# zhangxinsong-nlp/XFM

Hardware: AMD Instinct MI355X
Metric: image-text pairs/sec fwd+bwd, XFM-base 224px/30tok (higher is better)
Workload: dtype bf16; 1 GPU; Pretrain.py full multimodal step (ITC+ITM+MLM+MIM), XFM-base, synthetic 224px images + 30-token captions, random init; units_per_gpu=64, global_batch=64, dropout=True, ordered_reductions=True, grad_allreduce=False, parallelism=dp1, image_res=224

## Files before the change

xfm_amd/csrc/attention.hip:

```cpp
#include "attention_common.h"
#include "attention_general.hip"
#include "attention_short.hip"
#include "attention_grouped.hip"
#include "attention_vit.hip"
#include "attention_long.hip"
#include "attention_aux.hip"

static int attn_check(const AttnArgs& a, bool bwd) {
  XFM_REQUIRE(a.B > 0 && a.H > 0 && a.Sq > 0 && a.Sk > 0, "attention: empty problem B=%d H=%d Sq=%d Sk=%d", a.B, a.H, a.Sq, a.Sk);
  XFM_REQUIRE(a.q_rs % 8 == 0 && a.k_rs % 8 == 0 && a.v_rs % 8 == 0 && a.o_rs % 4 == 0, "attention: row strides must be multiples of 8");
  XFM_REQUIRE(((uintptr_t)a.q % 16) == 0 && ((uintptr_t)a.k % 16) == 0 && ((uintptr_t)a.v % 16) == 0 && ((uintptr_t)a.o % 8) == 0,
              "attention: q/k/v must be 16-byte aligned");
  XFM_REQUIRE(a.bias == nullptr || (a.bias_ld % 4 == 0 && a.bias_ld >= a.Sk), "attention: bias_ld must be a multiple of 4 and >= Sk");
  XFM_REQUIRE(a.B <= 65535 && a.H <= 65535, "attention: B/H exceed grid limits");
  XFM_REQUIRE(a.stat_ld >= a.Sq && a.stat_ld % 4 == 0 && ((uintptr_t)a.lse % 16) == 0, "attention: stat_ld must be a multiple of 4 and >= Sq, lse 16-byte aligned");
  XFM_REQUIRE(a.bias_t == nullptr || (a.bias != nullptr && a.bias_t_ld % 4 == 0 && a.bias_t_ld >= a.Sq), "attention: bad transposed bias");
  XFM_REQUIRE((a.q_start == nullptr) == (a.q_len == nullptr) && (a.k_start == nullptr) == (a.k_len == nullptr), "attention: packed rows need both start and len");
  XFM_REQUIRE((a.q_start == nullptr && a.k_start == nullptr) || (a.bias == nullptr && a.dbias == nullptr && a.kv_index == nullptr),
              "attention: packed rows take no additive bias and no kv_index");
  if (bwd) {
    XFM_REQUIRE(a.bwd_phase >= 0 && a.bwd_phase <= 2, "attention bwd: bwd_phase must be 0, 1 or 2");
    XFM_REQUIRE(a.dout && a.dq && a.dk && a.dv && a.delta && a.lse, "attention bwd: missing buffers");
    XFM_REQUIRE(a.do_rs % 8 == 0 && a.dq_rs % 4 == 0 && a.dk_rs % 4 == 0 && a.dv_rs % 4 == 0, "attention bwd: bad strides");
  }
  return XFM_OK;
}

static int attn_check_grouped(const AttnArgs& a) {
  XFM_REQUIRE(a.grp_rows != nullptr && a.n_groups > 0 && a.n_groups <= 65535, "grouped attention: grp_rows / n_groups missing");
  XFM_REQUIRE(a.Sq <= 64, "grouped attention needs Sq <= 64 (got %d)", a.Sq);
  XFM_REQUIRE(a.bias == nullptr && a.dbias == nullptr && a.causal == 0 && a.kv_index == nullptr,
              "grouped attention: no bias / causal mask / kv_index (the group index IS the key/value source)");
  XFM_REQUIRE(a.k_start == nullptr && a.k_len == nullptr, "grouped attention: only the query side may be packed (k_start / k_len must be NULL)");
  return XFM_OK;
}

int xfm_attn_fwd_impl(const AttnArgs& a, hipStream_t st) {
  int rc = attn_check(a, false);
  if (rc != XFM_OK) return rc;
  if (a.grp_start != nullptr) {
    rc = attn_check_grouped(a);
    return rc != XFM_OK ? rc : launch_xattn_fwd(a, st);
  }
  if (attn_packable(a)) return launch_xattn_fwd_packed(a, st);
  if (attn_vit_shape(a)) return launch_attn_fwd_vit(a, st);
  return launch_attn_fwd(a, st);
}

__global__ __launch_bounds__(256) void dbias_reduce_kernel(const float* __restrict__ ws, float* __restrict__ dbias, int B, long per_entry) {
  const long e = ((long)blockIdx.x * 256 + threadIdx.x) * 4;
  if (e >= per_entry) return;
  f32x4 acc = *reinterpret_cast<const f32x4*>(dbias + e);
  for (int b = 0; b < B; ++b) acc += *reinterpret_cast<const f32x4*>(ws + (long)b * per_entry + e);
  *reinterpret_cast<f32x4*>(dbias + e) = acc;
}

enum AttnDq { DQ_NONE, DQ_GROUPED, DQ_VIT, DQ_LONG, DQ_SHORT, DQ_SUMS, DQ_GENERAL };
enum AttnDkv { DKV_NONE, DKV_GROUPED, DKV_LONG, DKV_SHORT, DKV_GENERAL };
enum AttnDbias { DB_NONE, DB_ATOMICS, DB_SUMS, DB_ENTRY_WS, DB_SHORT_PLANES, DB_BLOCKS };
struct AttnBwdPlan {
  AttnDq dq;
  AttnDkv dkv;
  AttnDbias dbias;
  int nw, blocks;
  int groups, nb, slices;
  bool pre;
  int planes;
};

static bool xfm_deterministic() { return xfm_env_flag("XFM_DETERMINISTIC", false); }

static AttnBwdPlan attn_bwd_plan(const AttnArgs& a, bool have_ws) {
  AttnBwdPlan p = {};
  const bool run_dq = a.bwd_phase != 2, run_dkv = a.bwd_phase != 1;
  if (a.grp_start != nullptr) {
    if (run_dq) p.dq = DQ_GROUPED;
    if (run_dkv) p.dkv = DKV_GROUPED;
    return p;
  }
  const bool ws_ok = have_ws && a.dbias != nullptr && a.bias_ld % 4 == 0 && a.bias_ld <= (long)cdiv(a.Sk, 64) * 64 && a.q_start == nullptr;
  const int vit_mode = xfm_env_int("XFM_ATTN_VIT_BWD", 0);
  if (attn_vit3_shape(a, vit_mode)) {
    p.dq = DQ_VIT;
    if (a.dbias != nullptr) p.dbias = vit_mode == 4 && attn_dbias_blocks_ok(a) ? DB_BLOCKS : DB_ATOMICS;
  } else if (attn_long_shape(a)) {
    if (run_dq) {
      p.dq = DQ_LONG;
      if (a.dbias != nullptr) p.dbias = DB_BLOCKS;
    }
    if (run_dkv) p.dkv = attn_long_dkv_ok(a) ? DKV_LONG : DKV_GENERAL;
  } else {
    const bool short_ok = attn_short_dq_ok(a);
    attn_geom(a.Sq, p.nw, p.blocks);
    if (run_dq && short_ok) {
      p.dq = DQ_SHORT;
      p.slices = attn_short_dq_slices(a, p.groups, p.nb);
      p.pre = xfm_env_flag("XFM_ATTN_SHORT_PRE", false) && a.o != nullptr && a.o_lo != nullptr;
      if (a.dbias != nullptr) p.dbias = ws_ok && attn_short_planes_ok(a) && p.slices > 1 && xfm_deterministic() ? DB_SHORT_PLANES : DB_ATOMICS;
      if (p.dbias == DB_SHORT_PLANES) p.planes = p.slices;
    } else if (run_dq && a.dbias != nullptr && attn_resident(a.Sk, p.nw) && attn_plain(a)) {
      p.dq = DQ_SUMS;
      p.dbias = DB_SUMS;
      p.nb = attn_dbias_sums_nb(a, p.blocks);
    } else if (run_dq) {
      p.dq = DQ_GENERAL;
      if (a.dbias != nullptr) p.dbias = ws_ok && a.Sk > 64 * ATTN_RES_MAX ? DB_ENTRY_WS : DB_ATOMICS;
      if (p.dbias == DB_ENTRY_WS) p.planes = a.B;
    }
    if (run_dkv) p.dkv = short_ok && a.Sq <= 224 ? DKV_SHORT : DKV_GENERAL;
  }
  if (p.dbias == DB_BLOCKS) {
    p.slices = ws_ok ? attn_dbias_blocks_slices(a) : 1;
    p.planes = p.slices > 1 ? p.slices : 0;
  }
  return p;
}

long xfm_attn_bwd_workspace_impl(const AttnArgs& a) { return (long)attn_bwd_plan(a, true).planes * a.H * a.Sq * a.bias_ld * 4; }

#ifdef XFM_DIAG
static XfmTimeline attn_short_timeline = {nullptr, 0, 0};
static long long* attn_short_stamps(const AttnArgs& a, unsigned workgroups) {
  long long* dbg = a.Sk > 128 && a.Sk <= 224 ? attn_short_timeline.ptr : nullptr;
  if (dbg != nullptr && attn_short_timeline.bytes < (size_t)workgroups * XFM_ATTN_SHORT_STAMP_BYTES) {
    xfm_set_error("attn_bwd_dq_short: timeline buffer of %zu bytes is short of %u workgroups x %d: launched without stamps",
                  attn_short_timeline.bytes, workgroups, XFM_ATTN_SHORT_STAMP_BYTES);
    dbg = nullptr;
  }
  return dbg == nullptr ? dbg : reinterpret_cast<long long*>((uintptr_t)dbg | (uintptr_t)(attn_short_timeline.flags & 15));
}
#endif

int xfm_attn_bwd_impl(const AttnArgs& a_in, hipStream_t st) {
  int rc = attn_check(a_in, true);
  if (rc == XFM_OK && a_in.grp_start != nullptr) rc = attn_check_grouped(a_in);
  if (rc != XFM_OK) return rc;
  const AttnBwdPlan p = attn_bwd_plan(a_in, a_in.dbias_ws != nullptr);
  AttnArgs a = a_in;
  if (p.planes == 0) a.dbias_ws = nullptr;

  switch (p.dq) {
    case DQ_NONE: break;
    case DQ_GROUPED: rc = launch_xattn_dq(a, st); break;
    case DQ_VIT: {
      AttnArgs v = a;
      if (p.dbias == DB_BLOCKS) v.dbias = nullptr;
      rc = launch_attn_bwd_vit3(v, st);
      break;
    }
    case DQ_LONG: rc = launch_attn_bwd_long_dq(a, st); break;
    case DQ_SHORT:
#ifdef XFM_DIAG
      rc = launch_attn_bwd_dq_short(a, p.pre, p.groups, p.nb, p.slices, st, attn_short_stamps(a, (unsigned)(p.groups * a.H * p.slices)));
#else
      rc = launch_attn_bwd_dq_short(a, p.pre, p.groups, p.nb, p.slices, st);
#endif
      break;
    case DQ_SUMS: rc = launch_attn_bwd_dq(a, p.nw, p.blocks, p.nb, st); break;
    case DQ_GENERAL: rc = launch_attn_bwd_dq(a, p.nw, p.blocks, 0, st); break;
  }
  if (rc == XFM_OK && p.dbias == DB_BLOCKS) rc = launch_attn_dbias_blocks(a, p.slices, st);
  if (rc == XFM_OK && p.planes > 0) {
    const long per_entry = (long)a.H * a.Sq * a.bias_ld;
    hipLaunchKernelGGL(dbias_reduce_kernel, dim3(cdiv(per_entry / 4, 256)), dim3(256), 0, st, a.dbias_ws, a.dbias, p.planes, per_entry);
    rc = xfm_check_launch("dbias_reduce");
  }
  if (rc != XFM_OK) return rc;

  switch (p.dkv) {
    case DKV_NONE: break;
    case DKV_GROUPED: rc = launch_xattn_dkv(a, st); break;
    case DKV_LONG: rc = launch_attn_bwd_long_dkv(a, st); break;
    case DKV_SHORT: rc = launch_attn_bwd_dkv_short(a, st); break;
    case DKV_GENERAL: rc = launch_attn_bwd_dkv(a, st); break;
  }
  return rc;
}
```

xfm_amd/csrc/attention_general.hip:

```cpp
template <bool RES, bool PLAIN>
__global__ __launch_bounds__(1024) void attn_fwd_kernel(AttnArgs a) {
  extern __shared__ __attribute__((aligned(16))) char lds[];
  const int tid = threadIdx.x, lane = tid & 63, w = __builtin_amdgcn_readfirstlane(tid >> 6), nthreads = blockDim.x;
  const int lr = lane & 15, lg = lane >> 4;
  const int b = blockIdx.z, h = blockIdx.y;
  long qbase, kbase;
  int sq, sk;
  q_seq(a, b, qbase, sq);
  const int q0 = (blockIdx.x * (nthreads >> 6) + w) * 16;
  const bool wave_active = q0 < sq;
  const int qi = q0 + lr;
  const int qc = qi < sq ? qi : sq - 1;
  const uint32_t dkey = drop_key(a, b, h, qi);
  const bf16* qp = a.q + (qbase + qc) * a.q_rs + h * 64;
  const bf16x8 qf0 = *reinterpret_cast<const bf16x8*>(qp + 8 * lg);
  const bf16x8 qf1 = *reinterpret_cast<const bf16x8*>(qp + 32 + 8 * lg);
  const int kvb = a.kv_index ? a.kv_index[b] : b;
  k_seq(a, kvb, kbase, sk);
  const bf16* kb = a.k + kbase * a.k_rs + h * 64;
  const bf16* vb = a.v + kbase * a.v_rs + h * 64;

  f32x4 oacc[4];
#pragma unroll
  for (int i = 0; i < 4; ++i) oacc[i] = f32x4{0.f, 0.f, 0.f, 0.f};
  float m_run = EXCL_NEG, l_run = 0.f;

  const int nchunks = (sk + 63) / 64;
  constexpr bool resident = RES;
  const int nw = nthreads >> 6;
  if (resident) {
    for (int kc = 0; kc < nchunks; ++kc) stage_slot(lds + kc * ATTN_SLOT, kb, a.k_rs, vb, a.v_rs, kc * 64, sk, w, nw, lane);
    stage_wait();
  } else {
    stage_slot(lds, kb, a.k_rs, vb, a.v_rs, 0, sk, w, nw, lane);
  }
  for (int kc = 0; kc < nchunks; ++kc) {
    if (!resident) {
      stage_wait();
      if (kc + 1 < nchunks) stage_slot(lds + ((kc + 1) & 1) * ATTN_SLOT, kb, a.k_rs, vb, a.v_rs, (kc + 1) * 64, sk, w, nw, lane);
    }
    const char* sK = lds + (resident ? kc : (kc & 1)) * ATTN_SLOT;
    const char* sV = sK + ATTN_TILE;
    if (!wave_active) continue;
    f32x4 st[4], bvs[4];
    int kk[PLAIN ? 1 : 4][4];
    const bool has_mask = !PLAIN && a.key_keep != nullptr;
    const bool causal = !PLAIN && a.causal != 0;
    const bool plain = !has_mask && !causal && kc * 64 + 64 <= sk;
    load_bias(a, h, qc, kc, lg, bvs);
    if constexpr (!PLAIN) {
      if (has_mask) load_keep(a, kvb, kc, lg, kk);
    }
#pragma unroll
    for (int t = 0; t < 4; ++t) {
      st[t] = f32x4{0.f, 0.f, 0.f, 0.f};
      st[t] = __builtin_amdgcn_mfma_f32_16x16x32_bf16(row_frag(sK, t * 16, 0, lr, lg), qf0, st[t], 0, 0, 0);
      st[t] = __builtin_amdgcn_mfma_f32_16x16x32_bf16(row_frag(sK, t * 16, 1, lr, lg), qf1, st[t], 0, 0, 0);
    }
    float mx = EXCL_NEG;
    if (plain) {
#pragma unroll
      for (int t = 0; t < 4; ++t)
#pragma unroll
        for (int r = 0; r < 4; ++r) {
          st[t][r] = fmaf(st[t][r], a.scale, bvs[t][r]);
          mx = fmaxf(mx, st[t][r]);
        }
    } else {
#pragma unroll
      for (int t = 0; t < 4; ++t)
#pragma unroll
        for (int r = 0; r < 4; ++r) {
          st[t][r] = score_masked(a, st[t][r], bvs[t][r], has_mask, has_mask ? kk[PLAIN ? 0 : t][r] : 1, causal, qi, kc * 64 + t * 16 + 4 * lg + r, sk);
          mx = fmaxf(mx, st[t][r]);
        }
    }
    mx = group4_max(mx);
    const float m_new = fmaxf(m_run, mx);
    const float alpha = __expf(m_run - m_new);
    float psum = 0.f;
#pragma unroll
    for (int t = 0; t < 4; ++t)
#pragma unroll
      for (int r = 0; r < 4; ++r) {
        st[t][r] = __expf(st[t][r] - m_new);
        psum += st[t][r];
      }
    if (!PLAIN && a.drop_thresh != 0u) {
#pragma unroll
      for (int t = 0; t < 4; ++t)
#pragma unroll
        for (int r = 0; r < 4; ++r)
          st[t][r] = drop_keep(a, dkey, kc * 64 + t * 16 + 4 * lg + r) ? st[t][r] * a.drop_scale : 0.f;
    }
    psum = group4_sum(psum);
    l_run = l_run * alpha + psum;
    m_run = m_new;
#pragma unroll
    for (int dt = 0; dt < 4; ++dt)
#pragma unroll
      for (int r = 0; r < 4; ++r) oacc[dt][r] *= alpha;
#pragma unroll
    for (int s = 0; s < 2; ++s) {
      const bf16x8 pf = pack_pair(st[2 * s], st[2 * s + 1]);
#pragma unroll
      for (int dt = 0; dt < 4; ++dt)
        oacc[dt] = __builtin_amdgcn_mfma_f32_16x16x32_bf16(tr_frag(sV, 32 * s, 32 * s + 16, dt * 16, lr, lg), pf, oacc[dt], 0, 0, 0);
    }
  }
  if (!wave_active || qi >= sq) return;
  store_out(a, qbase + qi, h, lg, oacc, 1.0f / l_run);
  if (lg == 0) a.lse[((long)b * a.H + h) * a.stat_ld + qi] = m_run + __logf(l_run);
}

template <int NKC, bool RES, bool PLAIN>
__global__ __launch_bounds__(512) void attn_bwd_dq_kernel(AttnArgs a, int nb_per_block) {
  constexpr bool DBIAS = NKC > 0;
  constexpr int NACC = DBIAS ? NKC : 1;
  extern __shared__ __attribute__((aligned(16))) char lds[];
  const int tid = threadIdx.x, lane = tid & 63, w = __builtin_amdgcn_readfirstlane(tid >> 6), nthreads = blockDim.x;
  const int lr = lane & 15, lg = lane >> 4;
  const int h = blockIdx.y;
  const int q0 = (blockIdx.x * (nthreads >> 6) + w) * 16;
  const int qi = q0 + lr;
  constexpr bool resident = RES;

  f32x4 dsacc[NACC][4];
#pragma unroll
  for (int i = 0; i < NACC; ++i)
#pragma unroll
    for (int t = 0; t < 4; ++t) dsacc[i][t] = f32x4{0.f, 0.f, 0.f, 0.f};

  for (int bi = 0; bi < nb_per_block; ++bi) {
    const int b = blockIdx.z * nb_per_block + bi;
    if (b >= a.B) break;
    long qbase, kbase;
    int sq, sk;
    q_seq(a, b, qbase, sq);
    const bool wave_active = q0 < sq;
    const bool qvalid = qi < sq;
    const int qc = qvalid ? qi : sq - 1;
    const uint32_t dkey = drop_key(a, b, h, qi);
    const bf16* qp = a.q + (qbase + qc) * a.q_rs + h * 64;
    const bf16* dop = a.dout + (qbase + qc) * a.do_rs + h * 64;
    const bf16x8 qf0 = *reinterpret_cast<const bf16x8*>(qp + 8 * lg);
    const bf16x8 qf1 = *reinterpret_cast<const bf16x8*>(qp + 32 + 8 * lg);
    const bf16x8 df0 = *reinterpret_cast<const bf16x8*>(dop + 8 * lg);
    const bf16x8 df1 = *reinterpret_cast<const bf16x8*>(dop + 32 + 8 * lg);
    const long stat_idx = ((long)b * a.H + h) * a.stat_ld + qc;
    const float lse = a.lse[stat_idx];
    const int kvb = a.kv_index ? a.kv_index[b] : b;
    k_seq(a, kvb, kbase, sk);
    const int nchunks = (sk + 63) / 64;
    const bf16* kb = a.k + kbase * a.k_rs + h * 64;
    const bf16* vb = a.v + kbase * a.v_rs + h * 64;

    const int nw = nthreads >> 6;
    if (resident) {
      __syncthreads();
      for (int kc = 0; kc < nchunks; ++kc) stage_slot(lds + kc * ATTN_SLOT, kb, a.k_rs, vb, a.v_rs, kc * 64, sk, w, nw, lane);
      stage_wait();
    }
    auto stream_first = [&]() {
      __syncthreads();
      stage_slot(lds, kb, a.k_rs, vb, a.v_rs, 0, sk, w, nw, lane);
    };
    auto stream_next = [&](int kc) {
      stage_wait();
      if (kc + 1 < nchunks) stage_slot(lds + ((kc + 1) & 1) * ATTN_SLOT, kb, a.k_rs, vb, a.v_rs, (kc + 1) * 64, sk, w, nw, lane);
    };
    auto probs = [&](int kc, f32x4 (&st)[4], f32x4 (&dp)[4]) {
      const char* sK = lds + (resident ? kc : (kc & 1)) * ATTN_SLOT;
      const char* sV = sK + ATTN_TILE;
      f32x4 bvs[4];
      int kk[PLAIN ? 1 : 4][4];
      const bool has_mask = !PLAIN && a.key_keep != nullptr;
      const bool causal = !PLAIN && a.causal != 0;
      const bool plain = !has_mask && !causal && kc * 64 + 64 <= sk;
      load_bias(a, h, qc, kc, lg, bvs);
      if constexpr (!PLAIN) {
        if (has_mask) load_keep(a, kvb, kc, lg, kk);
      }
#pragma unroll
      for (int t = 0; t < 4; ++t) {
        st[t] = f32x4{0.f, 0.f, 0.f, 0.f};
        dp[t] = f32x4{0.f, 0.f, 0.f, 0.f};
        st[t] = __builtin_amdgcn_mfma_f32_16x16x32_bf16(row_frag(sK, t * 16, 0, lr, lg), qf0, st[t], 0, 0, 0);
        st[t] = __builtin_amdgcn_mfma_f32_16x16x32_bf16(row_frag(sK, t * 16, 1, lr, lg), qf1, st[t], 0, 0, 0);
        dp[t] = __builtin_amdgcn_mfma_f32_16x16x32_bf16(row_frag(sV, t * 16, 0, lr, lg), df0, dp[t], 0, 0, 0);
        dp[t] = __builtin_amdgcn_mfma_f32_16x16x32_bf16(row_frag(sV, t * 16, 1, lr, lg), df1, dp[t], 0, 0, 0);
      }
      const float lse_q = qvalid ? lse : 3.0e38f;
      if (plain) {
#pragma unroll
        for (int t = 0; t < 4; ++t)
#pragma unroll
          for (int r = 0; r < 4; ++r) st[t][r] = __expf(fmaf(st[t][r], a.scale, bvs[t][r]) - lse_q);
      } else {
#pragma unroll
        for (int t = 0; t < 4; ++t)
#pragma unroll
          for (int r = 0; r < 4; ++r)
            st[t][r] = __expf(score_masked(a, st[t][r], bvs[t][r], has_mask, has_mask ? kk[PLAIN ? 0 : t][r] : 1, causal, qi, kc * 64 + t * 16 + 4 * lg + r, sk) - lse_q);
      }
      if (!PLAIN && a.drop_thresh != 0u) {
#pragma unroll
        for (int t = 0; t < 4; ++t)
#pragma unroll
          for (int r = 0; r < 4; ++r)
            dp[t][r] = drop_keep(a, dkey, kc * 64 + t * 16 + 4 * lg + r) ? dp[t][r] * a.drop_scale : 0.f;
      }
    };

    float delta = 0.f;
    f32x4 st[4], dp[4];
    const bool fast_delta = a.o_lo != nullptr;
    if (fast_delta) {
      delta = delta_from_out(a, qbase + qc, h, lg, df0, df1);
    } else {
      if (!resident) stream_first();
      for (int kc = 0; kc < nchunks; ++kc) {
        if (!resident) stream_next(kc);
        if (wave_active) {
          probs(kc, st, dp);
#pragma unroll
          for (int t = 0; t < 4; ++t)
#pragma unroll
            for (int r = 0; r < 4; ++r) delta += st[t][r] * dp[t][r];
        }
      }
      delta = group4_sum(delta);
    }
    if (wave_active && qvalid && lg == 0) a.delta[stat_idx] = delta;

    f32x4 dqacc[4];
#pragma unroll
    for (int i = 0; i < 4; ++i) dqacc[i] = f32x4{0.f, 0.f, 0.f, 0.f};

    if (!resident && (nchunks > 1 || fast_delta)) stream_first();
    for (int kc = 0; kc < nchunks; ++kc) {
      if (nchunks > 1 || fast_delta) {
        if (!resident) stream_next(kc);
        if (wave_active) probs(kc, st, dp);
      }
      if (!wave_active) continue;
      const char* sK = lds + (resident ? kc : (kc & 1)) * ATTN_SLOT;
      float* wsrow = (!DBIAS && a.dbias != nullptr && a.dbias_ws != nullptr) ? a.dbias_ws + (((long)b * a.H + h) * a.Sq + qi) * a.bias_ld : nullptr;
#pragma unroll
      for (int t = 0; t < 4; ++t) {
        const int kj0 = kc * 64 + t * 16 + 4 * lg;
#pragma unroll
        for (int r = 0; r < 4; ++r) {
          const int kj = kj0 + r;
          const float ds = st[t][r] * (dp[t][r] - delta);
          st[t][r] = ds;
          if (!DBIAS && a.dbias != nullptr && wsrow == nullptr && kj < sk && qvalid) atomicAdd(a.dbias + ((long)h * a.Sq + qi) * a.bias_ld + kj, ds);
        }
        if (!DBIAS && wsrow != nullptr && qvalid) {
          if (kj0 + 4 <= a.bias_ld) *reinterpret_cast<f32x4*>(wsrow + kj0) = st[t];
          else
            for (int r = 0; r < 4; ++r)
              if (kj0 + r < a.bias_ld) wsrow[kj0 + r] = st[t][r];
        }
      }
      if (DBIAS) {
#pragma unroll
        for (int c = 0; c < NACC; ++c)
          if (c == kc) {
#pragma unroll
            for (int t = 0; t < 4; ++t) dsacc[c][t] += st[t];
          }
      }
#pragma unroll
      for (int s2 = 0; s2 < 2; ++s2) {
        const bf16x8 pf = pack_pair(st[2 * s2], st[2 * s2 + 1]);
#pragma unroll
        for (int dt = 0; dt < 4; ++dt)
          dqacc[dt] = __builtin_amdgcn_mfma_f32_16x16x32_bf16(tr_frag(sK, 32 * s2, 32 * s2 + 16, dt * 16, lr, lg), pf, dqacc[dt], 0, 0, 0);
      }
    }
    if (wave_active && qvalid) {
      bf16* dqp = a.dq + (qbase + qi) * a.dq_rs + h * 64;
#pragma unroll
      for (int dt = 0; dt < 4; ++dt) {
        bf16x4 ov;
#pragma unroll
        for (int r = 0; r < 4; ++r) ov[r] = f2bf(dqacc[dt][r] * a.scale);
        *reinterpret_cast<bf16x4*>(dqp + dt * 16 + 4 * lg) = ov;
      }
    }
  }

  if (DBIAS) {
    const bool wave_active = q0 < a.Sq;
    const int nchunks = (a.Sk + 63) / 64;
    float* fl = reinterpret_cast<float*>(lds + w * 4096);
#pragma unroll
    for (int kc = 0; kc < NACC; ++kc) {
      if (kc < nchunks) {
        __syncthreads();
#pragma unroll
        for (int t = 0; t < 4; ++t) *reinterpret_cast<f32x4*>(fl + lr * 64 + t * 16 + 4 * lg) = dsacc[kc][t];
        __syncthreads();
        if (wave_active && a.dbias != nullptr) {
          const int kj = kc * 64 + lane;
          for (int row = 0; row < 16; ++row) {
            const int q = q0 + row;
            if (q < a.Sq && kj < a.Sk) atomicAdd(a.dbias + ((long)h * a.Sq + q) * a.bias_ld + kj, fl[row * 64 + lane]);
          }
        }
      }
    }
  }
}

template <bool RES, bool PLAIN>
__global__ __launch_bounds__(512) void attn_bwd_dkv_kernel(AttnArgs a) {
  extern __shared__ __attribute__((aligned(16))) char lds[];
  const int tid = threadIdx.x, lane = tid & 63, w = __builtin_amdgcn_readfirstlane(tid >> 6), nthreads = blockDim.x;
  const int lr = lane & 15, lg = lane >> 4;
  const int b = blockIdx.z, h = blockIdx.y;
  const int kvb = a.kv_index ? a.kv_index[b] : b;
  long qbase, kbase, kout;
  int sq, sk, sk_unused;
  q_seq(a, b, qbase, sq);
  k_seq(a, kvb, kbase, sk);
  k_seq(a, b, kout, sk_unused);
  const int k0 = (blockIdx.x * (nthreads >> 6) + w) * 16;
  const bool wave_active = k0 < sk;
  const int kj = k0 + lr;
  const bool kvalid = kj < sk;
  const int kcl = kvalid ? kj : sk - 1;
  const bf16* kp = a.k + (kbase + kcl) * a.k_rs + h * 64;
  const bf16* vp = a.v + (kbase + kcl) * a.v_rs + h * 64;
  (void)sk_unused;
  const bf16x8 kf0 = *reinterpret_cast<const bf16x8*>(kp + 8 * lg);
  const bf16x8 kf1 = *reinterpret_cast<const bf16x8*>(kp + 32 + 8 * lg);
  const bf16x8 vf0 = *reinterpret_cast<const bf16x8*>(vp + 8 * lg);
  const bf16x8 vf1 = *reinterpret_cast<const bf16x8*>(vp + 32 + 8 * lg);
  const bf16* qb = a.q + qbase * a.q_rs + h * 64;
  const bf16* db = a.dout + qbase * a.do_rs + h * 64;
  const float* lse_b = a.lse + ((long)b * a.H + h) * a.stat_ld;
  const float* del_b = a.delta + ((long)b * a.H + h) * a.stat_ld;
  bool key_masked = false;
  if (!PLAIN && a.key_keep != nullptr) key_masked = a.key_keep[(long)kvb * a.Sk + kcl] == 0;
  const bool causal = !PLAIN && a.causal != 0;

  f32x4 dkacc[4], dvacc[4];
#pragma unroll
  for (int i = 0; i < 4; ++i) { dkacc[i] = f32x4{0.f, 0.f, 0.f, 0.f}; dvacc[i] = f32x4{0.f, 0.f, 0.f, 0.f}; }

  const int nchunks = (sq + 63) / 64;
  constexpr bool resident = RES;
  const int nw = nthreads >> 6;
  auto load_stats = [&](int step, f32x4 (&l)[2], f32x4 (&d)[2], f32x4 (&bt)[2]) {
#pragma unroll
    for (int u = 0; u < 2; ++u) {
      const int qi0 = step * 32 + u * 16 + 4 * lg;
      l[u] = d[u] = bt[u] = f32x4{0.f, 0.f, 0.f, 0.f};
      if (qi0 < a.Sq) {
        l[u] = *reinterpret_cast<const f32x4*>(lse_b + qi0);
        d[u] = *reinterpret_cast<const f32x4*>(del_b + qi0);
        if (a.bias_t != nullptr && kvalid) bt[u] = *reinterpret_cast<const f32x4*>(a.bias_t + ((long)h * a.Sk + kj) * a.bias_t_ld + qi0);
      }
    }
  };
  if (resident) {
    for (int qc = 0; qc < nchunks; ++qc) stage_slot(lds + qc * ATTN_SLOT, qb, a.q_rs, db, a.do_rs, qc * 64, sq, w, nw, lane);
    stage_wait();
  } else {
    stage_slot(lds, qb, a.q_rs, db, a.do_rs, 0, sq, w, nw, lane);
  }
  _Pragma("unroll 1") for (int qc = 0; qc < nchunks; ++qc) {
    if (!resident) {
      stage_wait();
      if (qc + 1 < nchunks) stage_slot(lds + ((qc + 1) & 1) * ATTN_SLOT, qb, a.q_rs, db, a.do_rs, (qc + 1) * 64, sq, w, nw, lane);
    }
    const char* sQ = lds + (resident ? qc : (qc & 1)) * ATTN_SLOT;
    const char* sD = sQ + ATTN_TILE;
    if (!wave_active) continue;
#pragma unroll
    for (int s2 = 0; s2 < 2; ++s2) {
      f32x4 st[2], dp[2], pd[2], lsev[2], delv[2], bvt[2];
      load_stats(qc * 2 + s2, lsev, delv, bvt);
#pragma unroll
      for (int u = 0; u < 2; ++u) {
        const int t = 2 * s2 + u;
        st[u] = f32x4{0.f, 0.f, 0.f, 0.f};
        dp[u] = f32x4{0.f, 0.f, 0.f, 0.f};
        st[u] = __builtin_amdgcn_mfma_f32_16x16x32_bf16(row_frag(sQ, t * 16, 0, lr, lg), kf0, st[u], 0, 0, 0);
        st[u] = __builtin_amdgcn_mfma_f32_16x16x32_bf16(row_frag(sQ, t * 16, 1, lr, lg), kf1, st[u], 0, 0, 0);
        dp[u] = __builtin_amdgcn_mfma_f32_16x16x32_bf16(row_frag(sD, t * 16, 0, lr, lg), vf0, dp[u], 0, 0, 0);
        dp[u] = __builtin_amdgcn_mfma_f32_16x16x32_bf16(row_frag(sD, t * 16, 1, lr, lg), vf1, dp[u], 0, 0, 0);
      }
      if (a.bias != nullptr && a.bias_t == nullptr) {
#pragma unroll
        for (int u = 0; u < 2; ++u)
#pragma unroll
          for (int r = 0; r < 4; ++r) {
            const int qi = qc * 64 + (2 * s2 + u) * 16 + 4 * lg + r;
            if (qi < a.Sq && kvalid) bvt[u][r] = a.bias[((long)h * a.Sq + qi) * a.bias_ld + kj];
          }
      }
      const float key_add = key_masked ? MASK_NEG : 0.f;
      const bool tail = qc * 64 + 64 > sq;
#pragma unroll
      for (int u = 0; u < 2; ++u) {
        const int qi0 = qc * 64 + (2 * s2 + u) * 16 + 4 * lg;
#pragma unroll
        for (int r = 0; r < 4; ++r) {
          const int qi = qi0 + r;
          float sc = fmaf(st[u][r], a.scale, bvt[u][r]);
          if (!PLAIN) sc += (causal & (kj > qi)) ? MASK_NEG : key_add;
          float pv = __expf(sc - lsev[u][r]);
          float dl = delv[u][r];
          if (tail) {
            pv = qi < sq ? pv : 0.f;
            dl = qi < sq ? dl : 0.f;
          }
          pv = kvalid ? pv : 0.f;
          delv[u][r] = dl;
          pd[u][r] = pv;
          st[u][r] = pv * (dp[u][r] - dl);
        }
      }
      if (!PLAIN && a.drop_thresh != 0u) {
#pragma unroll
        for (int u = 0; u < 2; ++u)
#pragma unroll
          for (int r = 0; r < 4; ++r) {
            const int qi = qc * 64 + (2 * s2 + u) * 16 + 4 * lg + r;
            const float keepf = drop_keep(a, drop_key(a, b, h, qi), kj) ? a.drop_scale : 0.f;
            st[u][r] = pd[u][r] * (dp[u][r] * keepf - delv[u][r]);
            pd[u][r] *= keepf;
          }
      }
      const bf16x8 pf = pack_pair(pd[0], pd[1]);
      const bf16x8 sf = pack_pair(st[0], st[1]);
#pragma unroll
      for (int dt = 0; dt < 4; ++dt) {
        dvacc[dt] = __builtin_amdgcn_mfma_f32_16x16x32_bf16(tr_frag(sD, 32 * s2, 32 * s2 + 16, dt * 16, lr, lg), pf, dvacc[dt], 0, 0, 0);
        dkacc[dt] = __builtin_amdgcn_mfma_f32_16x16x32_bf16(tr_frag(sQ, 32 * s2, 32 * s2 + 16, dt * 16, lr, lg), sf, dkacc[dt], 0, 0, 0);
      }
    }
  }
  if (!wave_active || !kvalid) return;
  bf16* dkp = a.dk + (kout + kj) * a.dk_rs + h * 64;
  bf16* dvp = a.dv + (kout + kj) * a.dv_rs + h * 64;
#pragma unroll
  for (int dt = 0; dt < 4; ++dt) {
    bf16x4 ok_, ov_;
#pragma unroll
    for (int r = 0; r < 4; ++r) { ok_[r] = f2bf(dkacc[dt][r] * a.scale); ov_[r] = f2bf(dvacc[dt][r]); }
    *reinterpret_cast<bf16x4*>(dkp + dt * 16 + 4 * lg) = ok_;
    *reinterpret_cast<bf16x4*>(dvp + dt * 16 + 4 * lg) = ov_;
  }
}

#define ATTN_RES_LDS (ATTN_RES_MAX * ATTN_SLOT)
#define ATTN_STREAM_LDS (2 * ATTN_SLOT)

static bool attn_resident(int S, int nw) { return cdiv(S, 64) <= ATTN_RES_MAX && nw >= 4; }

static size_t attn_lds_bytes(int S, int nw, size_t at_least) {
  size_t b = (size_t)(attn_resident(S, nw) ? cdiv(S, 64) : 2) * ATTN_SLOT;
  return b > at_least ? b : at_least;
}

static int launch_attn_fwd(const AttnArgs& a, hipStream_t st) {
  int nw, blocks;
  static const int fwd_nw = xfm_env_int("XFM_ATTN_FWD_NW", 8);
  attn_geom(a.Sq, nw, blocks, fwd_nw);
  const dim3 grid(blocks, a.H, a.B), blk(nw * 64);
  const size_t lds = attn_lds_bytes(a.Sk, nw, 0);
  if (attn_resident(a.Sk, nw)) {
    if (attn_plain(a)) lds_launch<attn_fwd_kernel<true, true>, ATTN_RES_LDS>(grid, blk, lds, st, a);
    else lds_launch<attn_fwd_kernel<true, false>, ATTN_RES_LDS>(grid, blk, lds, st, a);
  } else {
    if (attn_plain(a)) lds_launch<attn_fwd_kernel<false, true>, ATTN_STREAM_LDS>(grid, blk, lds, st, a);
    else lds_launch<attn_fwd_kernel<false, false>, ATTN_STREAM_LDS>(grid, blk, lds, st, a);
  }
  return xfm_check_launch("attn_fwd");
}

static int attn_dbias_sums_nb(const AttnArgs& a, int blocks) {
  int nb = a.B >= 8 ? 2 : 1;
  if (a.B >= 32) {
    const long c4 = (long)cdiv(blocks * a.H * cdiv(a.B, 4), 256) * 4, c8 = (long)cdiv(blocks * a.H * cdiv(a.B, 8), 256) * 8;
    nb = c8 <= c4 ? 8 : 4;
  }
  static const int nb_env = xfm_env_int("XFM_ATTN_DBIAS_NB", 0);
  return nb_env > 0 ? nb_env : nb;
}

static int launch_attn_bwd_dq(const AttnArgs& a, int nw, int blocks, int sums_nb, hipStream_t st) {
  const dim3 grid(blocks, a.H, sums_nb > 0 ? cdiv(a.B, sums_nb) : a.B), blk(nw * 64);
  const bool plain = attn_plain(a);
  if (sums_nb > 0) {
    lds_launch<attn_bwd_dq_kernel<4, true, true>, ATTN_RES_LDS>(grid, blk, attn_lds_bytes(a.Sk, nw, 8 * 4096), st, a, sums_nb);
  } else if (attn_resident(a.Sk, nw)) {
    if (plain) lds_launch<attn_bwd_dq_kernel<0, true, true>, ATTN_RES_LDS>(grid, blk, attn_lds_bytes(a.Sk, nw, 0), st, a, 1);
    else lds_launch<attn_bwd_dq_kernel<0, true, false>, ATTN_RES_LDS>(grid, blk, attn_lds_bytes(a.Sk, nw, 0), st, a, 1);
  } else {
    if (plain) lds_launch<attn_bwd_dq_kernel<0, false, true>, ATTN_STREAM_LDS>(grid, blk, attn_lds_bytes(a.Sk, nw, 0), st, a, 1);
    else lds_launch<attn_bwd_dq_kernel<0, false, false>, ATTN_STREAM_LDS>(grid, blk, attn_lds_bytes(a.Sk, nw, 0), st, a, 1);
  }
  return xfm_check_launch("attn_bwd_dq");
}

static int launch_attn_bwd_dkv(const AttnArgs& a, hipStream_t st) {
  int nw, blocks;
  attn_geom(a.Sk, nw, blocks);
  const dim3 grid(blocks, a.H, a.B), blk(nw * 64);
  const bool plain = attn_plain(a);
  static const bool dkv_res = xfm_env_flag("XFM_ATTN_DKV_RES", true);
  if (dkv_res && attn_resident(a.Sq, nw)) {
    if (plain) lds_launch<attn_bwd_dkv_kernel<true, true>, ATTN_RES_LDS>(grid, blk, attn_lds_bytes(a.Sq, nw, 0), st, a);
    else lds_launch<attn_bwd_dkv_kernel<true, false>, ATTN_RES_LDS>(grid, blk, attn_lds_bytes(a.Sq, nw, 0), st, a);
  } else {
    if (plain) lds_launch<attn_bwd_dkv_kernel<false, true>, ATTN_STREAM_LDS>(grid, blk, 2 * ATTN_SLOT, st, a);
    else lds_launch<attn_bwd_dkv_kernel<false, false>, ATTN_STREAM_LDS>(grid, blk, 2 * ATTN_SLOT, st, a);
  }
  return xfm_check_launch("attn_bwd_dkv");
}
```

Measured before the change: 1728 pairs/s.

## Add fused single-wave backward attention kernel for sequences up to 64

Adds a backward attention kernel that handles one (batch, head) problem per wave when Sq and Sk are at most 64 with no bias, causal mask or kv_index. It computes dQ, dK and dV in one pass, keeping Q, K and dO in LDS and holding the dK/dV accumulators in registers, and uses a smaller variant when both lengths are at most 32. This targets the 30-token text attention, replacing separate dq and dkv launches and their general tiling overhead. The new path only covers shapes the short kernel does not accept. It also duplicates masking, dropout and delta logic, which adds correctness risk.

```diff
diff --git a/xfm_amd/csrc/attention.hip b/xfm_amd/csrc/attention.hip
--- a/xfm_amd/csrc/attention.hip
+++ b/xfm_amd/csrc/attention.hip
@@ -55,8 +55,8 @@
   *reinterpret_cast<f32x4*>(dbias + e) = acc;
 }
 
-enum AttnDq { DQ_NONE, DQ_GROUPED, DQ_VIT, DQ_LONG, DQ_SHORT, DQ_SUMS, DQ_GENERAL };
-enum AttnDkv { DKV_NONE, DKV_GROUPED, DKV_LONG, DKV_SHORT, DKV_GENERAL };
+enum AttnDq { DQ_NONE, DQ_GROUPED, DQ_VIT, DQ_LONG, DQ_SHORT, DQ_SUMS, DQ_GENERAL, DQ_SMALL };
+enum AttnDkv { DKV_NONE, DKV_GROUPED, DKV_LONG, DKV_SHORT, DKV_GENERAL, DKV_SMALL };
 enum AttnDbias { DB_NONE, DB_ATOMICS, DB_SUMS, DB_ENTRY_WS, DB_SHORT_PLANES, DB_BLOCKS };
 struct AttnBwdPlan {
   AttnDq dq;
@@ -92,6 +92,11 @@
   } else {
     const bool short_ok = attn_short_dq_ok(a);
     attn_geom(a.Sq, p.nw, p.blocks);
+    if (!short_ok && attn_small_bwd_ok(a)) {
+      if (run_dq) p.dq = DQ_SMALL;
+      else p.dkv = DKV_SMALL;
+      return p;
+    }
     if (run_dq && short_ok) {
       p.dq = DQ_SHORT;
       p.slices = attn_short_dq_slices(a, p.groups, p.nb);
@@ -158,6 +163,7 @@
       break;
     case DQ_SUMS: rc = launch_attn_bwd_dq(a, p.nw, p.blocks, p.nb, st); break;
     case DQ_GENERAL: rc = launch_attn_bwd_dq(a, p.nw, p.blocks, 0, st); break;
+    case DQ_SMALL: rc = launch_attn_bwd_small(a, st); break;
   }
   if (rc == XFM_OK && p.dbias == DB_BLOCKS) rc = launch_attn_dbias_blocks(a, p.slices, st);
   if (rc == XFM_OK && p.planes > 0) {
@@ -173,6 +179,7 @@
     case DKV_LONG: rc = launch_attn_bwd_long_dkv(a, st); break;
     case DKV_SHORT: rc = launch_attn_bwd_dkv_short(a, st); break;
     case DKV_GENERAL: rc = launch_attn_bwd_dkv(a, st); break;
+    case DKV_SMALL: rc = launch_attn_bwd_small(a, st); break;
   }
   return rc;
 }
diff --git a/xfm_amd/csrc/attention_general.hip b/xfm_amd/csrc/attention_general.hip
--- a/xfm_amd/csrc/attention_general.hip
+++ b/xfm_amd/csrc/attention_general.hip
@@ -457,6 +457,220 @@
   }
 }
 
+#define SB_TILE(KT) ((KT) * 16 * 128)
+#define SB_WAVE_LDS(KT) (3 * SB_TILE(KT) + ((KT) == 2 ? 0 : 2 * 4096))
+#define SB_NW(KT) (4 / (KT))
+#define SB_LDS(KT) (SB_NW(KT) * SB_WAVE_LDS(KT))
+
+template <int KT>
+__device__ __forceinline__ void small_stage(char* tile, const bf16* g, long rs, int nvalid, int lane) {
+#pragma unroll
+  for (int j = 0; j < KT * 2; ++j) {
+    const int r = j * 8 + (lane >> 3);
+    const int c = (lane & 7) ^ swz_a(r);
+    const int gr = r < nvalid ? r : nvalid - 1;
+    lds_dma16(g + (long)gr * rs + c * 8, (unsigned)__builtin_amdgcn_readfirstlane((int)(uintptr_t)LDS_PTR(void, tile) + j * 1024));
+  }
+}
+
+template <int KT>
+__global__ __launch_bounds__(SB_NW(KT) * 64, KT == 2 ? 3 : 1) void attn_bwd_small_kernel(AttnArgs a) {
+  extern __shared__ __attribute__((aligned(16))) char lds[];
+  const int lane = threadIdx.x & 63, w = __builtin_amdgcn_readfirstlane(threadIdx.x >> 6);
+  const int lr = lane & 15, lg = lane >> 4;
+  const long prob = (long)blockIdx.x * SB_NW(KT) + w;
+  if (prob >= (long)a.B * a.H) return;
+  const int b = (int)(prob / a.H), h = (int)(prob - (long)b * a.H);
+  long qbase, kbase;
+  int sq, sk;
+  q_seq(a, b, qbase, sq);
+  k_seq(a, b, kbase, sk);
+  if (sq <= 0 || sk <= 0) return;
+  const bool want_dq = a.bwd_phase != 2, want_dkv = a.bwd_phase != 1;
+  char* sQ = lds + w * SB_WAVE_LDS(KT);
+  char* sK = sQ + SB_TILE(KT);
+  char* sD = sK + SB_TILE(KT);
+  char* sS = KT == 2 ? sK : sD + SB_TILE(KT);
+  char* sW = KT == 2 ? sS : sS + 4096;
+  constexpr int wcol = KT == 2 ? 32 : 0;
+
+  small_stage<KT>(sQ, a.q + qbase * a.q_rs + h * 64, a.q_rs, sq, lane);
+  small_stage<KT>(sK, a.k + kbase * a.k_rs + h * 64, a.k_rs, sk, lane);
+  small_stage<KT>(sD, a.dout + qbase * a.do_rs + h * 64, a.do_rs, sq, lane);
+  bf16x8 vf[KT][2];
+  const bf16* vb = a.v + kbase * a.v_rs + h * 64;
+#pragma unroll
+  for (int t = 0; t < KT; ++t) {
+    const int kr = t * 16 + lr < sk ? t * 16 + lr : sk - 1;
+    vf[t][0] = *reinterpret_cast<const bf16x8*>(vb + (long)kr * a.v_rs + 8 * lg);
+    vf[t][1] = *reinterpret_cast<const bf16x8*>(vb + (long)kr * a.v_rs + 32 + 8 * lg);
+  }
+  const bool has_mask = a.key_keep != nullptr;
+  unsigned kmasked = 0u;
+  if (has_mask) {
+    const int* row = a.key_keep + (long)b * a.Sk;
+#pragma unroll
+    for (int t = 0; t < KT; ++t)
+#pragma unroll
+      for (int r = 0; r < 4; ++r) {
+        const int kj = t * 16 + 4 * lg + r;
+        kmasked |= (row[kj < a.Sk ? kj : a.Sk - 1] == 0 ? 1u : 0u) << (4 * t + r);
+      }
+  }
+  const bool drop = a.drop_thresh != 0u;
+  const bool fast_delta = a.o_lo != nullptr;
+
+  f32x4 dkacc[4][KT], dvacc[4][KT];
+#pragma unroll
+  for (int dt = 0; dt < 4; ++dt)
+#pragma unroll
+    for (int kt = 0; kt < KT; ++kt) { dkacc[dt][kt] = f32x4{0.f, 0.f, 0.f, 0.f}; dvacc[dt][kt] = f32x4{0.f, 0.f, 0.f, 0.f}; }
+
+  asm volatile("s_waitcnt vmcnt(0)" ::: "memory");
+
+#pragma unroll
+  for (int qp = 0; qp < KT / 2; ++qp) {
+    if (qp * 32 >= sq) break;
+    bf16x4 dsv[2][KT], wv[2][KT];
+#pragma unroll
+    for (int u = 0; u < 2; ++u) {
+      const int q0 = qp * 32 + u * 16;
+#pragma unroll
+      for (int t = 0; t < KT; ++t) { dsv[u][t] = bf16x4{0, 0, 0, 0}; wv[u][t] = bf16x4{0, 0, 0, 0}; }
+      if (q0 < sq) {
+        const int qi = q0 + lr;
+        const bool qvalid = qi < sq;
+        const int qc = qvalid ? qi : sq - 1;
+        const long stat_idx = ((long)b * a.H + h) * a.stat_ld + qc;
+        const float lse = a.lse[stat_idx];
+        const float lse_q = qvalid ? lse : 3.0e38f;
+        float delta_in = 0.f;
+        if (!want_dq) delta_in = a.delta[stat_idx];
+        const uint32_t dkey = drop_key(a, b, h, qi);
+        const bf16x8 qf0 = row_frag(sQ, q0, 0, lr, lg), qf1 = row_frag(sQ, q0, 1, lr, lg);
+        const bf16x8 df0 = row_frag(sD, q0, 0, lr, lg), df1 = row_frag(sD, q0, 1, lr, lg);
+        f32x4 st[KT], dp[KT];
+#pragma unroll
+        for (int t = 0; t < KT; ++t) {
+          st[t] = f32x4{0.f, 0.f, 0.f, 0.f};
+          dp[t] = f32x4{0.f, 0.f, 0.f, 0.f};
+          st[t] = __builtin_amdgcn_mfma_f32_16x16x32_bf16(row_frag(sK, t * 16, 0, lr, lg), qf0, st[t], 0, 0, 0);
+          st[t] = __builtin_amdgcn_mfma_f32_16x16x32_bf16(row_frag(sK, t * 16, 1, lr, lg), qf1, st[t], 0, 0, 0);
+          dp[t] = __builtin_amdgcn_mfma_f32_16x16x32_bf16(vf[t][0], df0, dp[t], 0, 0, 0);
+          dp[t] = __builtin_amdgcn_mfma_f32_16x16x32_bf16(vf[t][1], df1, dp[t], 0, 0, 0);
+        }
+        float wscale[KT][4];
+#pragma unroll
+        for (int t = 0; t < KT; ++t)
+#pragma unroll
+          for (int r = 0; r < 4; ++r) {
+            const int kj = t * 16 + 4 * lg + r;
+            st[t][r] = __expf(score_masked(a, st[t][r], 0.f, has_mask, (int)(~kmasked >> (4 * t + r)) & 1, false, qi, kj, sk) - lse_q);
+            wscale[t][r] = 1.f;
+            if (drop) {
+              const bool keep = drop_keep(a, dkey, kj);
+              wscale[t][r] = keep ? a.drop_scale : 0.f;
+              dp[t][r] = keep ? dp[t][r] * a.drop_scale : 0.f;
+            }
+          }
+        float delta;
+        if (!want_dq) {
+          delta = qvalid ? delta_in : 0.f;
+        } else if (fast_delta) {
+          delta = delta_from_out(a, qbase + qc, h, lg, df0, df1);
+        } else {
+          delta = 0.f;
+#pragma unroll
+          for (int t = 0; t < KT; ++t)
+#pragma unroll
+            for (int r = 0; r < 4; ++r) delta += st[t][r] * dp[t][r];
+          delta = group4_sum(delta);
+        }
+        if (want_dq && qvalid && lg == 0) a.delta[stat_idx] = delta;
+#pragma unroll
+        for (int t = 0; t < KT; ++t)
+#pragma unroll
+          for (int r = 0; r < 4; ++r) {
+            const float pv = st[t][r];
+            st[t][r] = pv * (dp[t][r] - delta);
+            dsv[u][t][r] = f2bf(st[t][r]);
+            wv[u][t][r] = f2bf(pv * wscale[t][r]);
+          }
+        if (want_dq) {
+          f32x4 dqacc[4];
+#pragma unroll
+          for (int dt = 0; dt < 4; ++dt) dqacc[dt] = f32x4{0.f, 0.f, 0.f, 0.f};
+#pragma unroll
+          for (int s2 = 0; s2 < KT / 2; ++s2) {
+            const bf16x8 pf = pack_pair(st[2 * s2], st[2 * s2 + 1]);
+#pragma unroll
+            for (int dt = 0; dt < 4; ++dt)
+              dqacc[dt] = __builtin_amdgcn_mfma_f32_16x16x32_bf16(tr_frag(sK, 32 * s2, 32 * s2 + 16, dt * 16, lr, lg), pf, dqacc[dt], 0, 0, 0);
+          }
+          if (qvalid) {
+            bf16* dqp = a.dq + (qbase + qi) * a.dq_rs + h * 64;
+#pragma unroll
+            for (int dt = 0; dt < 4; ++dt) {
+              bf16x4 ov;
+#pragma unroll
+              for (int r = 0; r < 4; ++r) ov[r] = f2bf(dqacc[dt][r] * a.scale);
+              *reinterpret_cast<bf16x4*>(dqp + dt * 16 + 4 * lg) = ov;
+            }
+          }
+        }
+      }
+    }
+    if (want_dkv) {
+      asm volatile("s_waitcnt lgkmcnt(0)" ::: "memory");
+#pragma unroll
+      for (int u = 0; u < 2; ++u) {
+        const int row = u * 16 + lr;
+#pragma unroll
+        for (int t = 0; t < KT; ++t) {
+          const int cs = t * 16 + 4 * lg, cw = wcol + cs;
+          *reinterpret_cast<bf16x4*>(sS + row * 128 + (((cs >> 3) ^ swz_a(row)) << 4) + (cs & 7) * 2) = dsv[u][t];
+          *reinterpret_cast<bf16x4*>(sW + row * 128 + (((cw >> 3) ^ swz_a(row)) << 4) + (cw & 7) * 2) = wv[u][t];
+        }
+      }
+      asm volatile("s_waitcnt lgkmcnt(0)" ::: "memory");
+      bf16x8 sf[KT], wf[KT];
+#pragma unroll
+      for (int kt = 0; kt < KT; ++kt) {
+        sf[kt] = tr_frag(sS, 0, 16, kt * 16, lr, lg);
+        wf[kt] = tr_frag(sW, 0, 16, wcol + kt * 16, lr, lg);
+      }
+#pragma unroll
+      for (int dt = 0; dt < 4; ++dt) {
+        const bf16x8 qt = tr_frag(sQ, qp * 32, qp * 32 + 16, dt * 16, lr, lg);
+        const bf16x8 dot = tr_frag(sD, qp * 32, qp * 32 + 16, dt * 16, lr, lg);
+#pragma unroll
+        for (int kt = 0; kt < KT; ++kt) {
+          dkacc[dt][kt] = __builtin_amdgcn_mfma_f32_16x16x32_bf16(qt, sf[kt], dkacc[dt][kt], 0, 0, 0);
+          dvacc[dt][kt] = __builtin_amdgcn_mfma_f32_16x16x32_bf16(dot, wf[kt], dvacc[dt][kt], 0, 0, 0);
+        }
+      }
+      asm volatile("s_waitcnt lgkmcnt(0)" ::: "memory");
+    }
+  }
+  if (!want_dkv) return;
+#pragma unroll
+  for (int kt = 0; kt < KT; ++kt) {
+    const int kj = kt * 16 + lr;
+    if (kj < sk) {
+      bf16* dkp = a.dk + (kbase + kj) * a.dk_rs + h * 64;
+      bf16* dvp = a.dv + (kbase + kj) * a.dv_rs + h * 64;
+#pragma unroll
+      for (int dt = 0; dt < 4; ++dt) {
+        bf16x4 ok_, ov_;
+#pragma unroll
+        for (int r = 0; r < 4; ++r) { ok_[r] = f2bf(dkacc[dt][kt][r] * a.scale); ov_[r] = f2bf(dvacc[dt][kt][r]); }
+        *reinterpret_cast<bf16x4*>(dkp + dt * 16 + 4 * lg) = ok_;
+        *reinterpret_cast<bf16x4*>(dvp + dt * 16 + 4 * lg) = ov_;
+      }
+    }
+  }
+}
+
 #define ATTN_RES_LDS (ATTN_RES_MAX * ATTN_SLOT)
 #define ATTN_STREAM_LDS (2 * ATTN_SLOT)
 
@@ -523,3 +737,15 @@
   }
   return xfm_check_launch("attn_bwd_dkv");
 }
+
+static bool attn_small_bwd_ok(const AttnArgs& a) {
+  return xfm_env_flag("XFM_ATTN_SMALL_BWD", true) && a.Sq <= 64 && a.Sk <= 64 && a.bias == nullptr && a.dbias == nullptr && a.causal == 0 &&
+         a.kv_index == nullptr && (long)a.B * a.H <= (1L << 30);
+}
+
+static int launch_attn_bwd_small(const AttnArgs& a, hipStream_t st) {
+  const long probs = (long)a.B * a.H;
+  if (a.Sq <= 32 && a.Sk <= 32) lds_launch<attn_bwd_small_kernel<2>, SB_LDS(2)>(dim3(cdiv(probs, SB_NW(2))), dim3(SB_NW(2) * 64), SB_LDS(2), st, a);
+  else lds_launch<attn_bwd_small_kernel<4>, SB_LDS(4)>(dim3(cdiv(probs, SB_NW(4))), dim3(SB_NW(4) * 64), SB_LDS(4), st, a);
+  return xfm_check_launch("attn_bwd_small");
+}
```

After: 1607 pairs/s. 7.0% lower.
